# soon-yau/upgpt

Hardware: AMD Instinct MI355X
Metric: 256x256 images/sec, 50-step DDIM, bs=8/GPU; UNet MFMA util % (higher is better)
Workload: dtype f16; 1 GPU; BASELINE configs[1]: bs=8/GPU, 256x256 px (latent 4x32x32), 50-step DDIM eta=0, text-only cond [B,87,768], UNet(bbox.yaml) + VAE decode, EMA weights, no CFG; batch_per_gpu=8, ddim_steps=50, batches_in_flight_per_gpu=4, lane_hw_queues=measured, parallelism=replica-dp1, one all-gather of images per batch

## Files before the change

### upgpt_amd/csrc/attention.hip

```cpp
#include <stdlib.h>

#include "common.h"

namespace {

struct AttnArgs {
  const f16* q;
  const f16* k;
  const f16* vt;
  f16* o;
  int ldq, ldk, vt_ld, ldo;
  long qbs, kbs, obs;
  int heads, nq, nkv;
  float scale_log2;
  int causal;
};

__device__ __forceinline__ float raw_exp2(float x) { return __builtin_amdgcn_exp2f(x); }
__device__ __forceinline__ float max_over_key_groups(float x) {
  unsigned u = __float_as_uint(x);
  const auto a = __builtin_amdgcn_permlane32_swap(u, u, false, false);
  u = __float_as_uint(fmaxf(__uint_as_float(a[0]), __uint_as_float(a[1])));
  const auto b = __builtin_amdgcn_permlane16_swap(u, u, false, false);
  return fmaxf(__uint_as_float(b[0]), __uint_as_float(b[1]));
}
__device__ __forceinline__ float sum_over_key_groups(float x) {
  unsigned u = __float_as_uint(x);
  const auto a = __builtin_amdgcn_permlane32_swap(u, u, false, false);
  u = __float_as_uint(__uint_as_float(a[0]) + __uint_as_float(a[1]));
  const auto b = __builtin_amdgcn_permlane16_swap(u, u, false, false);
  return __uint_as_float(b[0]) + __uint_as_float(b[1]);
}
#define ATT_ONES ((f16x8){(f16)1.f, (f16)1.f, (f16)1.f, (f16)1.f, (f16)1.f, (f16)1.f, (f16)1.f, (f16)1.f})

template <int D, int QREG, int NS, int QT>
__device__ __forceinline__ void attn_tile(const AttnArgs& a, const f16* const* qrow, const bool* q_ok,
                                          const f16x8 (*qf)[QREG ? D / 32 : 1], const f16* kbase,
                                          const f16* vbase, int kb, int g, int c, f32x4 (*o)[D / 16], float* mrun,
                                          f32x4* lsum, int q0) {
  constexpr int KD = D / 32;
  constexpr int DT = D / 16;
  constexpr int NC = NS / 2;
  const f16x8 zero8 = {0, 0, 0, 0, 0, 0, 0, 0};
  f32x4 s[QT][NS];
  const f16* kp[NS];
#pragma unroll
  for (int t = 0; t < NS; ++t) {
    const int key = kb + 16 * t + c;
    kp[t] = kbase + (long)(key < a.nkv ? key : 0) * a.ldk;
#pragma unroll
    for (int u = 0; u < QT; ++u) s[u][t] = (f32x4){0.f, 0.f, 0.f, 0.f};
  }
#pragma unroll
  for (int kd = 0; kd < KD; ++kd) {
    f16x8 qv[QT];
#pragma unroll
    for (int u = 0; u < QT; ++u)
      qv[u] = QREG ? qf[u][kd] : (q_ok[u] ? *(const f16x8*)(qrow[u] + kd * 32) : zero8);
#pragma unroll
    for (int t = 0; t < NS; ++t) {
      const f16x8 kf = *(const f16x8*)(kp[t] + kd * 32);
#pragma unroll
      for (int u = 0; u < QT; ++u) s[u][t] = __builtin_amdgcn_mfma_f32_16x16x32_f16(kf, qv[u], s[u][t], 0, 0, 0);
    }
  }
  constexpr bool VPRE = (D <= 128);
  f16x4 vpre[VPRE ? DT * NC * 2 : 1];
  if (VPRE) {
#pragma unroll
    for (int i = 0; i < DT; ++i)
#pragma unroll
      for (int j = 0; j < NC; ++j) {
        const f16* vr = vbase + (long)i * 16 * a.vt_ld + kb + 32 * j;
        vpre[(i * NC + j) * 2] = *(const f16x4*)vr;
        vpre[(i * NC + j) * 2 + 1] = *(const f16x4*)(vr + 16);
      }
  }
  const float cs = a.scale_log2;
  f16x8 pf[QT][NC];
  const bool tail = kb + NS * 16 > a.nkv;
#pragma unroll
  for (int u = 0; u < QT; ++u) {
    if (tail || a.causal) {
      const int qlim = a.causal ? q0 + u * 16 + c : a.nkv;
#pragma unroll
      for (int t = 0; t < NS; ++t)
#pragma unroll
        for (int r = 0; r < 4; ++r) {
          const int key = kb + 16 * t + 4 * g + r;
          if (key >= a.nkv || key > qlim) s[u][t][r] = -INFINITY;
        }
    }
    float mx = -INFINITY;
#pragma unroll
    for (int t = 0; t < NS; ++t)
      mx = fmaxf(mx, fmaxf(fmaxf(s[u][t][0], s[u][t][1]), fmaxf(s[u][t][2], s[u][t][3])));
    mx = max_over_key_groups(mx);
    const float mnew = fmaxf(mrun[u], mx);
    if (__builtin_amdgcn_ballot_w64(mnew != mrun[u]) != 0) {
      const float alpha = raw_exp2((mrun[u] - mnew) * cs);
      lsum[u] *= alpha;
#pragma unroll
      for (int i = 0; i < DT; ++i) o[u][i] *= alpha;
    }
    mrun[u] = mnew;
    const float mc = -mnew * cs;
#pragma unroll
    for (int t = 0; t < NS; ++t)
#pragma unroll
      for (int r = 0; r < 4; ++r) pf[u][t >> 1][(t & 1) * 4 + r] = (f16)raw_exp2(fmaf(s[u][t][r], cs, mc));
  }
#pragma unroll
  for (int j = 0; j < NC; ++j)
#pragma unroll
    for (int u = 0; u < QT; ++u) lsum[u] = __builtin_amdgcn_mfma_f32_16x16x32_f16(ATT_ONES, pf[u][j], lsum[u], 0, 0, 0);
#pragma unroll
  for (int i = 0; i < DT; ++i)
#pragma unroll
    for (int j = 0; j < NC; ++j) {
      f16x4 va, vb;
      if (VPRE) {
        va = vpre[(i * NC + j) * 2];
        vb = vpre[(i * NC + j) * 2 + 1];
      } else {
        const f16* vr = vbase + (long)i * 16 * a.vt_ld + kb + 32 * j;
        va = *(const f16x4*)vr;
        vb = *(const f16x4*)(vr + 16);
      }
      const f16x8 vf = {va[0], va[1], va[2], va[3], vb[0], vb[1], vb[2], vb[3]};
#pragma unroll
      for (int u = 0; u < QT; ++u) o[u][i] = __builtin_amdgcn_mfma_f32_16x16x32_f16(vf, pf[u][j], o[u][i], 0, 0, 0);
    }
}

template <int D, int QREG, int QT>
__global__ __launch_bounds__(256) void attn_kernel(const AttnArgs a) {
  constexpr int KD = D / 32;
  constexpr int DT = D / 16;
  const int lane = threadIdx.x & 63;
  const int wave = threadIdx.x >> 6;
  const int g = lane >> 4, c = lane & 15;
  const int bh = blockIdx.x;
#ifndef UPK_NO_XCD_SAMPLE
  const int nb_ = gridDim.x / a.heads;
  const int b = bh % nb_;
  const int h = bh / nb_;
#else
  const int b = bh / a.heads;
  const int h = bh - b * a.heads;
#endif
  const int q0 = (blockIdx.y * (blockDim.x >> 6) + wave) * 16 * QT;
  if (q0 >= a.nq) return;
  const f16* kbase = a.k + b * a.kbs + h * D + g * 8;
  const f16* vbase = a.vt + ((long)(b * a.heads + h) * D + c) * a.vt_ld + g * 4;
  const f16x8 zero8 = {0, 0, 0, 0, 0, 0, 0, 0};

  const f16* qrow[QT];
  bool q_ok[QT];
  f16x8 qf[QT][QREG ? KD : 1];
  f32x4 o[QT][DT];
  float mrun[QT];
  f32x4 lsum[QT];
#pragma unroll
  for (int u = 0; u < QT; ++u) {
    const int qi = q0 + u * 16 + c;
    q_ok[u] = qi < a.nq;
    qrow[u] = a.q + b * a.qbs + (long)(q_ok[u] ? qi : 0) * a.ldq + h * D + g * 8;
    if (QREG) {
#pragma unroll
      for (int kd = 0; kd < KD; ++kd) qf[u][kd] = q_ok[u] ? *(const f16x8*)(qrow[u] + kd * 32) : zero8;
    }
#pragma unroll
    for (int i = 0; i < DT; ++i) o[u][i] = (f32x4){0.f, 0.f, 0.f, 0.f};
    mrun[u] = -INFINITY;
    lsum[u] = (f32x4){0.f, 0.f, 0.f, 0.f};
  }

  int kb = 0;
  if (D <= 128) {
    for (; kb + 64 <= (a.causal ? min(a.nkv, q0 + 16 * QT) : a.nkv); kb += 64)
      attn_tile<D, QREG, 4, QT>(a, qrow, q_ok, qf, kbase, vbase, kb, g, c, o, mrun, lsum, q0);
  }
  const int kend = a.causal ? min(a.nkv, q0 + 16 * QT) : a.nkv;
  for (; kb < kend; kb += 32) attn_tile<D, QREG, 2, QT>(a, qrow, q_ok, qf, kbase, vbase, kb, g, c, o, mrun, lsum, q0);

#pragma unroll
  for (int u = 0; u < QT; ++u) {
    const float inv = 1.0f / lsum[u][0];
    if (!q_ok[u]) continue;
    f16* orow = a.o + b * a.obs + (long)(q0 + u * 16 + c) * a.ldo + h * D + g * 4;
#pragma unroll
    for (int i = 0; i < DT; ++i) {
      f16x4 ov;
#pragma unroll
      for (int r = 0; r < 4; ++r) ov[r] = (f16)(o[u][i][r] * inv);
      *(f16x4*)(orow + i * 16) = ov;
    }
  }
}

struct QProj {
  const f16* x;
  const f16* w;
  const float* u;
  const float* bias;
  long xbs;
  int ldx, cq, ln_dim;
  float eps;
};

template <int D, int QT>
__global__ __launch_bounds__(256) void attn_qproj_kernel(const AttnArgs a, const QProj p) {
  constexpr int KD = D / 32;
  constexpr int DT = D / 16;
  constexpr int KC = 7;
  const int lane = threadIdx.x & 63;
  const int wave = threadIdx.x >> 6;
  const int g = lane >> 4, c = lane & 15;
  const int bh = blockIdx.y;
  const int b = bh / a.heads;
  const int h = bh - b * a.heads;
  const int q0 = (blockIdx.x * (blockDim.x >> 6) + wave) * 16 * QT;
  if (q0 >= a.nq) return;
  const f16* kbase = a.k + b * a.kbs + h * D + g * 8;
  const f16* vbase = a.vt + ((long)(b * a.heads + h) * D + c) * a.vt_ld + g * 4;

  const f16* qrow[QT];
  bool q_ok[QT];
  f16x8 qf[QT][KD];
  f32x4 o[QT][DT];
  float mrun[QT];
  f32x4 lsum[QT];
  {
    f32x4 qa[QT][DT];
    float s1[QT], s2[QT];
    const f16* xr[QT];
#pragma unroll
    for (int u = 0; u < QT; ++u) {
      const int qi = q0 + u * 16 + c;
      q_ok[u] = qi < a.nq;
      qrow[u] = nullptr;
      xr[u] = p.x + b * p.xbs + (long)(q_ok[u] ? qi : 0) * p.ldx + g * 8;
      s1[u] = s2[u] = 0.f;
#pragma unroll
      for (int i = 0; i < DT; ++i) qa[u][i] = (f32x4){0.f, 0.f, 0.f, 0.f};
    }
    const f16* wr = p.w + (long)(h * D + c) * p.cq + g * 8;
    const long wtile = (long)16 * p.cq;
    const f16x2 one2 = {(f16)1.f, (f16)1.f};
    for (int k0 = 0; k0 < p.cq; k0 += KC * 32) {
      f16x8 xv[QT][KC], wv[DT][KC];
#pragma unroll
      for (int kc = 0; kc < KC; ++kc) {
#pragma unroll
        for (int u = 0; u < QT; ++u) xv[u][kc] = *(const f16x8*)(xr[u] + k0 + kc * 32);
#pragma unroll
        for (int i = 0; i < DT; ++i) wv[i][kc] = *(const f16x8*)(wr + i * wtile + k0 + kc * 32);
      }
#pragma unroll
      for (int kc = 0; kc < KC; ++kc) {
#pragma unroll
        for (int u = 0; u < QT; ++u) {
#pragma unroll
          for (int hh = 0; hh < 4; ++hh) {
            const f16x2 xx = {xv[u][kc][2 * hh], xv[u][kc][2 * hh + 1]};
            s1[u] = __builtin_amdgcn_fdot2(xx, one2, s1[u], false);
            s2[u] = __builtin_amdgcn_fdot2(xx, xx, s2[u], false);
          }
#pragma unroll
          for (int i = 0; i < DT; ++i)
            qa[u][i] = __builtin_amdgcn_mfma_f32_16x16x32_f16(wv[i][kc], xv[u][kc], qa[u][i], 0, 0, 0);
        }
      }
    }
    const float inv_dim = 1.0f / (float)p.ln_dim;
    float mean[QT], rstd[QT];
#pragma unroll
    for (int u = 0; u < QT; ++u) {
      const float t1 = sum_over_key_groups(s1[u]), t2 = sum_over_key_groups(s2[u]);
      mean[u] = t1 * inv_dim;
      rstd[u] = rsqrtf(fmaxf(t2 * inv_dim - mean[u] * mean[u], 0.f) + p.eps);
    }
#pragma unroll
    for (int kd = 0; kd < KD; ++kd) {
      const int d0 = h * D + kd * 32 + g * 8;
      const f32x4 u0 = *(const f32x4*)(p.u + d0), u1 = *(const f32x4*)(p.u + d0 + 4);
      const f32x4 b0 = *(const f32x4*)(p.bias + d0), b1 = *(const f32x4*)(p.bias + d0 + 4);
#pragma unroll
      for (int u = 0; u < QT; ++u)
#pragma unroll
        for (int r = 0; r < 4; ++r) {
          qf[u][kd][r] = (f16)((qa[u][2 * kd][r] - mean[u] * u0[r]) * rstd[u] + b0[r]);
          qf[u][kd][4 + r] = (f16)((qa[u][2 * kd + 1][r] - mean[u] * u1[r]) * rstd[u] + b1[r]);
        }
    }
  }
#pragma unroll
  for (int u = 0; u < QT; ++u) {
#pragma unroll
    for (int i = 0; i < DT; ++i) o[u][i] = (f32x4){0.f, 0.f, 0.f, 0.f};
    mrun[u] = -INFINITY;
    lsum[u] = (f32x4){0.f, 0.f, 0.f, 0.f};
  }
  int kb = 0;
  for (; kb + 64 <= a.nkv; kb += 64) attn_tile<D, 1, 4, QT>(a, qrow, q_ok, qf, kbase, vbase, kb, g, c, o, mrun, lsum, q0);
  for (; kb < a.nkv; kb += 32) attn_tile<D, 1, 2, QT>(a, qrow, q_ok, qf, kbase, vbase, kb, g, c, o, mrun, lsum, q0);
#pragma unroll
  for (int u = 0; u < QT; ++u) {
    const float inv = 1.0f / lsum[u][0];
    if (!q_ok[u]) continue;
    f16* orow = a.o + b * a.obs + (long)(q0 + u * 16 + c) * a.ldo + h * D + g * 4;
#pragma unroll
    for (int i = 0; i < DT; ++i) {
      f16x4 ov;
#pragma unroll
      for (int r = 0; r < 4; ++r) ov[r] = (f16)(o[u][i][r] * inv);
      *(f16x4*)(orow + i * 16) = ov;
    }
  }
}

constexpr int ATT_VROW = 72;
__device__ __forceinline__ int att_swz(int row, int chunk) { return chunk ^ ((-(row >> 2)) & 3); }

template <int D, int QT>
__global__ __launch_bounds__(256) void attn_lds_kernel(const AttnArgs a) {
  constexpr int KD = D / 32;
  constexpr int DT = D / 16;
  __shared__ __attribute__((aligned(16))) f16 sk[2][KD * 64 * 32];
  __shared__ __attribute__((aligned(16))) f16 sv[2][D * ATT_VROW];
  const int tid = threadIdx.x;
  const int lane = tid & 63, wave = tid >> 6;
  const int g = lane >> 4, c = lane & 15;
  const int bh = blockIdx.x;
#ifndef UPK_NO_XCD_SAMPLE
  const int nb_ = gridDim.x / a.heads;
  const int b = bh % nb_;
  const int h = bh / nb_;
#else
  const int b = bh / a.heads;
  const int h = bh - b * a.heads;
#endif
  const int q0 = (blockIdx.y * 4 + wave) * 16 * QT;
  const f16x8 zero8 = {0, 0, 0, 0, 0, 0, 0, 0};

  bool q_ok[QT];
  f16x8 qf[QT][KD];
  f32x4 o[QT][DT];
  float mrun[QT];
  f32x4 lsum[QT];
#pragma unroll
  for (int u = 0; u < QT; ++u) {
    const int qi = q0 + u * 16 + c;
    q_ok[u] = qi < a.nq;
    const f16* qrow = a.q + b * a.qbs + (long)(q_ok[u] ? qi : 0) * a.ldq + h * D + g * 8;
#pragma unroll
    for (int kd = 0; kd < KD; ++kd) qf[u][kd] = q_ok[u] ? *(const f16x8*)(qrow + kd * 32) : zero8;
#pragma unroll
    for (int i = 0; i < DT; ++i) o[u][i] = (f32x4){0.f, 0.f, 0.f, 0.f};
    mrun[u] = -INFINITY;
    lsum[u] = (f32x4){0.f, 0.f, 0.f, 0.f};
  }
  const f16* ksrc = a.k + b * a.kbs + (long)(tid >> 2) * a.ldk + h * D + (tid & 3) * 8;
  const f16* vsrc = a.vt + ((long)(b * a.heads + h) * D + (tid >> 3)) * a.vt_ld + (tid & 7) * 8;
  const int kdst = (tid >> 2) * 32 + att_swz(tid >> 2, tid & 3) * 8;
  const int vdst = (tid >> 3) * ATT_VROW + (tid & 7) * 8;
  f16x8 kreg[KD], vreg[KD];
  auto fetch = [&](int kb) {
#pragma unroll
    for (int it = 0; it < KD; ++it) {
      kreg[it] = *(const f16x8*)(ksrc + (long)kb * a.ldk + it * 32);
      vreg[it] = *(const f16x8*)(vsrc + (long)it * 32 * a.vt_ld + kb);
    }
  };
  auto stash = [&](int buf) {
#pragma unroll
    for (int it = 0; it < KD; ++it) {
      *(f16x8*)(&sk[buf][it * 64 * 32 + kdst]) = kreg[it];
      *(f16x8*)(&sv[buf][it * 32 * ATT_VROW + vdst]) = vreg[it];
    }
  };
  const int ntiles = a.nkv >> 6;
  fetch(0);
  stash(0);
  __syncthreads();
  const float cs = a.scale_log2;
  const int kfrag = c * 32 + att_swz(c, g) * 8;
  for (int t = 0; t < ntiles; ++t) {
    const int buf = t & 1;
    if (t + 1 < ntiles) fetch((t + 1) << 6);
    f32x4 sc[QT][4];
#pragma unroll
    for (int tt = 0; tt < 4; ++tt)
#pragma unroll
      for (int u = 0; u < QT; ++u) sc[u][tt] = (f32x4){0.f, 0.f, 0.f, 0.f};
#pragma unroll
    for (int kd = 0; kd < KD; ++kd)
#pragma unroll
      for (int tt = 0; tt < 4; ++tt) {
        const f16x8 kf = *(const f16x8*)(&sk[buf][(kd * 64 + tt * 16) * 32 + kfrag]);
#pragma unroll
        for (int u = 0; u < QT; ++u) sc[u][tt] = __builtin_amdgcn_mfma_f32_16x16x32_f16(kf, qf[u][kd], sc[u][tt], 0, 0, 0);
      }
    f16x8 pf[QT][2];
#pragma unroll
    for (int u = 0; u < QT; ++u) {
      float mx = -INFINITY;
#pragma unroll
      for (int tt = 0; tt < 4; ++tt)
        mx = fmaxf(mx, fmaxf(fmaxf(sc[u][tt][0], sc[u][tt][1]), fmaxf(sc[u][tt][2], sc[u][tt][3])));
      mx = max_over_key_groups(mx);
      const float mnew = fmaxf(mrun[u], mx);
      if (__builtin_amdgcn_ballot_w64(mnew != mrun[u]) != 0) {
        const float alpha = raw_exp2((mrun[u] - mnew) * cs);
        lsum[u] *= alpha;
#pragma unroll
        for (int i = 0; i < DT; ++i) o[u][i] *= alpha;
      }
      mrun[u] = mnew;
      const float mc = -mnew * cs;
#pragma unroll
      for (int tt = 0; tt < 4; ++tt)
#pragma unroll
        for (int r = 0; r < 4; ++r) pf[u][tt >> 1][(tt & 1) * 4 + r] = (f16)raw_exp2(fmaf(sc[u][tt][r], cs, mc));
    }
#pragma unroll
    for (int j = 0; j < 2; ++j)
#pragma unroll
      for (int u = 0; u < QT; ++u) lsum[u] = __builtin_amdgcn_mfma_f32_16x16x32_f16(ATT_ONES, pf[u][j], lsum[u], 0, 0, 0);
#pragma unroll
    for (int i = 0; i < DT; ++i)
#pragma unroll
      for (int j = 0; j < 2; ++j) {
        const f16* vr = &sv[buf][(i * 16 + c) * ATT_VROW + 32 * j + 4 * g];
        const f16x4 va = *(const f16x4*)vr, vb = *(const f16x4*)(vr + 16);
        const f16x8 vf = {va[0], va[1], va[2], va[3], vb[0], vb[1], vb[2], vb[3]};
#pragma unroll
        for (int u = 0; u < QT; ++u) o[u][i] = __builtin_amdgcn_mfma_f32_16x16x32_f16(vf, pf[u][j], o[u][i], 0, 0, 0);
      }
    if (t + 1 < ntiles) stash(buf ^ 1);
    __syncthreads();
  }
#pragma unroll
  for (int u = 0; u < QT; ++u) {
    const float inv = 1.0f / lsum[u][0];
    if (!q_ok[u]) continue;
    f16* orow = a.o + b * a.obs + (long)(q0 + u * 16 + c) * a.ldo + h * D + g * 4;
#pragma unroll
    for (int i = 0; i < DT; ++i) {
      f16x4 ov;
#pragma unroll
      for (int r = 0; r < 4; ++r) ov[r] = (f16)(o[u][i][r] * inv);
      *(f16x4*)(orow + i * 16) = ov;
    }
  }
}

}

static int attn_waves_per_block(const upk_ctx* ctx, int bh, int n_q, int qt) {
  static const int wpb_env = getenv("UPK_ATTN_WPB") ? atoi(getenv("UPK_ATTN_WPB")) : 0;
  if (wpb_env == 1 || wpb_env == 2 || wpb_env == 4) return wpb_env;
  int wpb = 4;
  while (wpb > 1 && (long)bh * ((n_q + 16 * qt * wpb - 1) / (16 * qt * wpb)) < 2L * ctx->num_cus) wpb >>= 1;
  return wpb;
}

template <int D>
__global__ __launch_bounds__(256) void attn_wide_kernel(const AttnArgs a) {
  typedef __attribute__((address_space(3))) void* lds_ptr;
  typedef const __attribute__((address_space(1))) void* glb_ptr;
  constexpr int KD = D / 32, DT = D / 16;
  constexpr int KROW = D * 2 + 32;
  constexpr int KBYTES = 32 * KROW;
  constexpr int VBYTES = D * 64;
  constexpr int BUF = KBYTES + VBYTES;
  extern __shared__ __attribute__((aligned(16))) char smem[];
  const int lane = threadIdx.x & 63, wave = __builtin_amdgcn_readfirstlane(threadIdx.x >> 6);
  const int g = lane >> 4, c = lane & 15;
  const int b = blockIdx.x;
  const int q0 = (blockIdx.y * 4 + wave) * 16;
  const f16* kg = a.k + b * a.kbs;
  const f16* vg = a.vt + (long)b * D * a.vt_ld;
  auto issue = [&](int kb, int buf) {
    char* base = smem + buf * BUF;
#pragma unroll
    for (int i = 0; i < 8; ++i) {
      const int r = wave + 4 * i;
      const f16* src = kg + (long)(kb + r) * a.ldk + lane * 8;
      __builtin_amdgcn_global_load_lds((glb_ptr)src, (lds_ptr)(base + r * KROW), 16, 0, 0);
    }
#pragma unroll
    for (int i = 0; i < D / 64; ++i) {
      const int rb = (wave + 4 * i) * 16;
      const int row = rb + (lane >> 2), pc = (lane & 3) ^ ((row >> 2) & 3);
      const f16* src = vg + (long)row * a.vt_ld + kb + pc * 8;
      __builtin_amdgcn_global_load_lds((glb_ptr)src, (lds_ptr)(base + KBYTES + rb * 64), 16, 0, 0);
    }
  };
  issue(0, 0);
  const bool q_ok = q0 + c < a.nq;
  const f16* qrow = a.q + b * a.qbs + (long)(q_ok ? q0 + c : 0) * a.ldq + g * 8;
  f16x8 qf[KD];
#pragma unroll
  for (int kd = 0; kd < KD; ++kd) qf[kd] = q_ok ? *(const f16x8*)(qrow + kd * 32) : (f16x8){0, 0, 0, 0, 0, 0, 0, 0};
  f32x4 o[DT];
#pragma unroll
  for (int i = 0; i < DT; ++i) o[i] = (f32x4){0.f, 0.f, 0.f, 0.f};
  f32x4 lsum = {0.f, 0.f, 0.f, 0.f};
  float mrun = -INFINITY;
  const float cs = a.scale_log2;
  const int ntiles = a.nkv >> 5;
  const int vsw = (c >> 2) & 3;
  for (int t = 0; t < ntiles; ++t) {
    const int buf = t & 1;
    asm volatile("s_waitcnt vmcnt(0)" ::: "memory");
    __syncthreads();
    if (t + 1 < ntiles) issue((t + 1) << 5, buf ^ 1);
    const char* kt = smem + buf * BUF + c * KROW + g * 16;
    const char* vt = smem + buf * BUF + KBYTES + c * 64;
    f32x4 sc[2];
#pragma unroll
    for (int tt = 0; tt < 2; ++tt) {
      sc[tt] = (f32x4){0.f, 0.f, 0.f, 0.f};
#pragma unroll
      for (int kd = 0; kd < KD; ++kd) {
        const f16x8 kf = *(const f16x8*)(kt + tt * 16 * KROW + kd * 64);
        sc[tt] = __builtin_amdgcn_mfma_f32_16x16x32_f16(kf, qf[kd], sc[tt], 0, 0, 0);
      }
    }
    float mx = fmaxf(fmaxf(fmaxf(sc[0][0], sc[0][1]), fmaxf(sc[0][2], sc[0][3])),
                     fmaxf(fmaxf(sc[1][0], sc[1][1]), fmaxf(sc[1][2], sc[1][3])));
    mx = max_over_key_groups(mx);
    const float mnew = fmaxf(mrun, mx);
    if (__builtin_amdgcn_ballot_w64(mnew != mrun) != 0) {
      const float alpha = raw_exp2((mrun - mnew) * cs);
      lsum *= alpha;
#pragma unroll
      for (int i = 0; i < DT; ++i) o[i] *= alpha;
    }
    mrun = mnew;
    const float mc = -mnew * cs;
    f16x8 pf;
#pragma unroll
    for (int tt = 0; tt < 2; ++tt)
#pragma unroll
      for (int r = 0; r < 4; ++r) pf[tt * 4 + r] = (f16)raw_exp2(fmaf(sc[tt][r], cs, mc));
    lsum = __builtin_amdgcn_mfma_f32_16x16x32_f16(ATT_ONES, pf, lsum, 0, 0, 0);
#pragma unroll
    for (int i = 0; i < DT; ++i) {
      const char* vr = vt + i * 16 * 64 + (g & 1) * 8;
      const f16x4 va = *(const f16x4*)(vr + (((g >> 1) ^ vsw) << 4));
      const f16x4 vb = *(const f16x4*)(vr + (((2 + (g >> 1)) ^ vsw) << 4));
      const f16x8 vf = {va[0], va[1], va[2], va[3], vb[0], vb[1], vb[2], vb[3]};
      o[i] = __builtin_amdgcn_mfma_f32_16x16x32_f16(vf, pf, o[i], 0, 0, 0);
    }
  }
  if (!q_ok) return;
  const float inv = 1.0f / lsum[0];
  f16* orow = a.o + b * a.obs + (long)(q0 + c) * a.ldo + g * 4;
#pragma unroll
  for (int i = 0; i < DT; ++i) {
    f16x4 ov;
#pragma unroll
    for (int r = 0; r < 4; ++r) ov[r] = (f16)(o[i][r] * inv);
    *(f16x4*)(orow + i * 16) = ov;
  }
}

static int attention_impl(upk_ctx* ctx, const void* q, int ldq, long long qbs, const void* k, int ldk, long long kbs,
                          const void* vt, int vt_ld, void* out, int ldo, long long obs, int batch, int heads, int n_q,
                          int n_kv, int d, float scale, int causal, upk_stream stream_) {
  if (!ctx) return UPK_EINVAL;
  if (!q || !k || !vt || !out) return upk_fail(ctx, UPK_EINVAL, "attention: null pointer");
  if (batch <= 0 || heads <= 0 || n_q <= 0 || n_kv <= 0) return upk_fail(ctx, UPK_EINVAL, "attention: empty");
  if ((ldq & 7) || (ldk & 7) || (vt_ld & 3) || (ldo & 3) || vt_ld < ((n_kv + 31) & ~31))
    return upk_fail(ctx, UPK_EINVAL, "attention: ldq/ldk %% 8, vt_ld %% 4 and vt_ld >= round_up(n_kv,32) required");
  hipStream_t stream = (hipStream_t)stream_;
  AttnArgs a;
  a.q = (const f16*)q;
  a.k = (const f16*)k;
  a.vt = (const f16*)vt;
  a.o = (f16*)out;
  a.ldq = ldq;
  a.ldk = ldk;
  a.vt_ld = vt_ld;
  a.ldo = ldo;
  a.qbs = qbs;
  a.kbs = kbs;
  a.obs = obs;
  a.heads = heads;
  a.nq = n_q;
  a.nkv = n_kv;
  a.scale_log2 = scale * 1.4426950408889634f;
  a.causal = causal;
  if (causal && n_q != n_kv) return upk_fail(ctx, UPK_EINVAL, "attention: causal needs n_q == n_kv");
  static const int qt_env = getenv("UPK_ATTN_QT") ? atoi(getenv("UPK_ATTN_QT")) : 0;
  const int qt = qt_env ? qt_env : ((d <= 128 && (long)((n_q + 127) / 128) * batch * heads >= 4L * ctx->num_cus) ? 2 : 1);
  dim3 grid(batch * heads, (n_q + 64 * qt - 1) / (64 * qt)), block(256);
  upk_prof_scope prof(ctx, UPK_CLS_ATTN, stream);
  static const bool lds_off = getenv("UPK_ATTN_DIRECT") != nullptr;
  if (!lds_off && !causal && (d == 32 || d == 64) && n_kv >= 256 && (n_kv & 63) == 0 && (vt_ld & 7) == 0) {
    if (d == 32) {
      if (qt == 2) hipLaunchKernelGGL((attn_lds_kernel<32, 2>), grid, block, 0, stream, a);
      else hipLaunchKernelGGL((attn_lds_kernel<32, 1>), grid, block, 0, stream, a);
    } else {
      if (qt == 2) hipLaunchKernelGGL((attn_lds_kernel<64, 2>), grid, block, 0, stream, a);
      else hipLaunchKernelGGL((attn_lds_kernel<64, 1>), grid, block, 0, stream, a);
    }
    return upk_check_launch(ctx, "attention_lds");
  }
  {
    const int wpb = attn_waves_per_block(ctx, batch * heads, n_q, d <= 128 ? qt : 1);
    if (d <= 128) {
      grid = dim3(batch * heads, (n_q + 16 * qt * wpb - 1) / (16 * qt * wpb));
      block = dim3(64 * wpb);
    }
  }
#define UPK_ATTN(D_, QR_)                                                                         \
  if (qt == 2)                                                                                    \
    hipLaunchKernelGGL((attn_kernel<D_, QR_, (D_ <= 128 ? 2 : 1)>), grid, block, 0, stream, a);  \
  else                                                                                            \
    hipLaunchKernelGGL((attn_kernel<D_, QR_, 1>), grid, block, 0, stream, a);
  switch (d) {
    case 32: UPK_ATTN(32, 1) break;
    case 64: UPK_ATTN(64, 1) break;
    case 128: UPK_ATTN(128, 1) break;
    case 512:
      static const bool wide_off = getenv("UPK_ATTN_WIDE_OFF") != nullptr;
      if (heads == 1 && !causal && (n_kv & 31) == 0 && ldk >= 512 && !wide_off &&
          ((ldk | ldq | vt_ld) & 7) == 0 && ((kbs | qbs) & 7) == 0 &&
          (((uintptr_t)q | (uintptr_t)k | (uintptr_t)vt) & 15) == 0) {
        static unsigned long long wide_mask = 0;
        int rcw = upk_lds_attr_once(ctx, (const void*)attn_wide_kernel<512>, &wide_mask);
        if (rcw != UPK_OK) return rcw;
        const size_t lds = 2 * (32 * (512 * 2 + 32) + 512 * 64);
        hipLaunchKernelGGL((attn_wide_kernel<512>), dim3(batch, (n_q + 63) / 64), dim3(256), lds, stream, a);
        return upk_check_launch(ctx, "attention_wide");
      }
      [[fallthrough]];
    case 256: {
      const int wpb = attn_waves_per_block(ctx, batch * heads, n_q, 1);
      const dim3 g2(batch * heads, (n_q + 16 * wpb - 1) / (16 * wpb)), b2(64 * wpb);
      if (d == 256) hipLaunchKernelGGL((attn_kernel<256, 1, 1>), g2, b2, 0, stream, a);
      else hipLaunchKernelGGL((attn_kernel<512, 0, 1>), g2, b2, 0, stream, a);
      break;
    }
    default: return upk_fail(ctx, UPK_ESHAPE, "attention: head dim %d not in {32,64,128,256,512}", d);
  }
#undef UPK_ATTN
  return upk_check_launch(ctx, "attention");
}

extern "C" int upk_attention_f16(upk_ctx* ctx, const void* q, int ldq, long long qbs, const void* k, int ldk,
                                 long long kbs, const void* vt, int vt_ld, void* out, int ldo, long long obs,
                                 int batch, int heads, int n_q, int n_kv, int d, float scale, upk_stream stream) {
  return attention_impl(ctx, q, ldq, qbs, k, ldk, kbs, vt, vt_ld, out, ldo, obs, batch, heads, n_q, n_kv, d, scale, 0,
                        stream);
}

extern "C" int upk_attention_causal_f16(upk_ctx* ctx, const void* q, int ldq, long long qbs, const void* k, int ldk,
                                        long long kbs, const void* vt, int vt_ld, void* out, int ldo, long long obs,
                                        int batch, int heads, int n, int d, float scale, upk_stream stream) {
  return attention_impl(ctx, q, ldq, qbs, k, ldk, kbs, vt, vt_ld, out, ldo, obs, batch, heads, n, n, d, scale, 1, stream);
}

extern "C" int upk_attention_qproj_f16(upk_ctx* ctx, const void* x, int ldx, long long xbs, int cq, int ln_dim,
                                       float ln_eps, const void* wq, const float* wq_colsum, const float* wq_bias,
                                       const void* k, int ldk, long long kbs, const void* vt, int vt_ld, void* out,
                                       int ldo, long long obs, int batch, int heads, int n_q, int n_kv, int d,
                                       float scale, upk_stream stream_) {
  if (!ctx) return UPK_EINVAL;
  if (!x || !wq || !wq_colsum || !wq_bias || !k || !vt || !out) return upk_fail(ctx, UPK_EINVAL, "attention_qproj: null pointer");
  if (batch <= 0 || heads <= 0 || n_q <= 0 || n_kv <= 0) return upk_fail(ctx, UPK_EINVAL, "attention_qproj: empty");
  if ((ldx & 7) || (ldk & 7) || (vt_ld & 3) || (ldo & 3) || vt_ld < ((n_kv + 31) & ~31))
    return upk_fail(ctx, UPK_EINVAL, "attention_qproj: ldx/ldk %% 8, vt_ld %% 4 and vt_ld >= round_up(n_kv,32) required");
  if ((d != 32 && d != 64) || cq <= 0 || cq % 224 || ln_dim <= 0 || ln_dim > cq || ldx < cq)
    return upk_fail(ctx, UPK_ESHAPE, "attention_qproj: head dim %d / %d input channels outside {32,64} / 224*n", d, cq);
  hipStream_t stream = (hipStream_t)stream_;
  AttnArgs a;
  a.q = nullptr;
  a.k = (const f16*)k;
  a.vt = (const f16*)vt;
  a.o = (f16*)out;
  a.ldq = 0;
  a.ldk = ldk;
  a.vt_ld = vt_ld;
  a.ldo = ldo;
  a.qbs = 0;
  a.kbs = kbs;
  a.obs = obs;
  a.heads = heads;
  a.nq = n_q;
  a.nkv = n_kv;
  a.scale_log2 = scale * 1.4426950408889634f;
  a.causal = 0;
  QProj p;
  p.x = (const f16*)x;
  p.w = (const f16*)wq;
  p.u = wq_colsum;
  p.bias = wq_bias;
  p.xbs = xbs;
  p.ldx = ldx;
  p.cq = cq;
  p.ln_dim = ln_dim;
  p.eps = ln_eps;
  upk_prof_scope prof(ctx, UPK_CLS_ATTN, stream);
  const int qt = d == 32 ? 2 : 1;
  const int wpb = attn_waves_per_block(ctx, batch * heads, n_q, qt);
  const dim3 grid((n_q + 16 * qt * wpb - 1) / (16 * qt * wpb), batch * heads), block(64 * wpb);
  if (d == 32) hipLaunchKernelGGL((attn_qproj_kernel<32, 2>), grid, block, 0, stream, a, p);
  else hipLaunchKernelGGL((attn_qproj_kernel<64, 1>), grid, block, 0, stream, a, p);
  return upk_check_launch(ctx, "attention_qproj");
}
```

Before: 98.94 images/s.

## Software-pipeline LDS attention kernel with swizzled V layout and multi-tile stages

Restructures the LDS flash-attention kernel so the next tile's QK scores and V fragments are loaded while the current tile's PV accumulation runs, using ping-pong register sets. For D=32 it stages two 64-key tiles per barrier (four LDS slots) to halve synchronisation. V in LDS now uses an XOR-swizzled 64-wide row instead of padded 72-wide rows, so each V fragment is a single 16-byte read. It also lowers the threshold for picking QT=2 on the LDS path. Costs are higher register pressure and more LDS for D=32, which may reduce occupancy.

Result: no change. 98.76 images/s (median of 2 runs) (-0.2%).

```diff
diff --git a/upgpt_amd/csrc/attention.hip b/upgpt_amd/csrc/attention.hip
--- a/upgpt_amd/csrc/attention.hip
+++ b/upgpt_amd/csrc/attention.hip
@@ -320,15 +320,17 @@
   }
 }
 
-constexpr int ATT_VROW = 72;
+constexpr int ATT_VROW = 64;
 __device__ __forceinline__ int att_swz(int row, int chunk) { return chunk ^ ((-(row >> 2)) & 3); }
 
 template <int D, int QT>
 __global__ __launch_bounds__(256) void attn_lds_kernel(const AttnArgs a) {
   constexpr int KD = D / 32;
   constexpr int DT = D / 16;
-  __shared__ __attribute__((aligned(16))) f16 sk[2][KD * 64 * 32];
-  __shared__ __attribute__((aligned(16))) f16 sv[2][D * ATT_VROW];
+  constexpr int TPS = D == 32 ? 2 : 1;
+  constexpr int NSLOT = 2 * TPS;
+  __shared__ __attribute__((aligned(16))) f16 sk[NSLOT][KD * 64 * 32];
+  __shared__ __attribute__((aligned(16))) f16 sv[NSLOT][D * ATT_VROW];
   const int tid = threadIdx.x;
   const int lane = tid & 63, wave = tid >> 6;
   const int g = lane >> 4, c = lane & 15;
@@ -364,32 +366,46 @@
   const f16* ksrc = a.k + b * a.kbs + (long)(tid >> 2) * a.ldk + h * D + (tid & 3) * 8;
   const f16* vsrc = a.vt + ((long)(b * a.heads + h) * D + (tid >> 3)) * a.vt_ld + (tid & 7) * 8;
   const int kdst = (tid >> 2) * 32 + att_swz(tid >> 2, tid & 3) * 8;
-  const int vdst = (tid >> 3) * ATT_VROW + (tid & 7) * 8;
-  f16x8 kreg[KD], vreg[KD];
-  auto fetch = [&](int kb) {
-#pragma unroll
-    for (int it = 0; it < KD; ++it) {
-      kreg[it] = *(const f16x8*)(ksrc + (long)kb * a.ldk + it * 32);
-      vreg[it] = *(const f16x8*)(vsrc + (long)it * 32 * a.vt_ld + kb);
+  const int vrow = tid >> 3, vj = (tid & 7) >> 2, vw = (tid & 3) * 8;
+  const int vq = 4 * vj + (vw & 15) / 4, vh = vw >> 4;
+  const int vdst0 = vrow * ATT_VROW + ((vq ^ (vrow & 7)) << 3) + 4 * vh;
+  const int vdst1 = vrow * ATT_VROW + (((vq + 1) ^ (vrow & 7)) << 3) + 4 * vh;
+  const int ntiles = a.nkv >> 6;
+  const int nstages = (ntiles + TPS - 1) / TPS;
+  f16x8 kreg[TPS][KD], vreg[TPS][KD];
+  auto fetch = [&](int st) {
+#pragma unroll
+    for (int j = 0; j < TPS; ++j) {
+      const int kb = (st * TPS + j) << 6;
+      if (TPS == 1 || kb < a.nkv) {
+#pragma unroll
+        for (int it = 0; it < KD; ++it) {
+          kreg[j][it] = *(const f16x8*)(ksrc + (long)kb * a.ldk + it * 32);
+          vreg[j][it] = *(const f16x8*)(vsrc + (long)it * 32 * a.vt_ld + kb);
+        }
+      }
     }
   };
-  auto stash = [&](int buf) {
-#pragma unroll
-    for (int it = 0; it < KD; ++it) {
-      *(f16x8*)(&sk[buf][it * 64 * 32 + kdst]) = kreg[it];
-      *(f16x8*)(&sv[buf][it * 32 * ATT_VROW + vdst]) = vreg[it];
+  auto stash = [&](int st) {
+#pragma unroll
+    for (int j = 0; j < TPS; ++j) {
+      const int tl = st * TPS + j;
+      if (TPS == 1 || tl < ntiles) {
+        const int slot = tl % NSLOT;
+#pragma unroll
+        for (int it = 0; it < KD; ++it) {
+          *(f16x8*)(&sk[slot][it * 64 * 32 + kdst]) = kreg[j][it];
+          const f16x8 vv = vreg[j][it];
+          *(f16x4*)(&sv[slot][it * 32 * ATT_VROW + vdst0]) = (f16x4){vv[0], vv[1], vv[2], vv[3]};
+          *(f16x4*)(&sv[slot][it * 32 * ATT_VROW + vdst1]) = (f16x4){vv[4], vv[5], vv[6], vv[7]};
+        }
+      }
     }
   };
-  const int ntiles = a.nkv >> 6;
-  fetch(0);
-  stash(0);
-  __syncthreads();
   const float cs = a.scale_log2;
   const int kfrag = c * 32 + att_swz(c, g) * 8;
-  for (int t = 0; t < ntiles; ++t) {
-    const int buf = t & 1;
-    if (t + 1 < ntiles) fetch((t + 1) << 6);
-    f32x4 sc[QT][4];
+  auto load_tile = [&](int tl, f32x4 (&sc)[QT][4], f16x8 (&vf)[DT][2]) {
+    const int slot = tl % NSLOT;
 #pragma unroll
     for (int tt = 0; tt < 4; ++tt)
 #pragma unroll
@@ -398,11 +414,19 @@
     for (int kd = 0; kd < KD; ++kd)
 #pragma unroll
       for (int tt = 0; tt < 4; ++tt) {
-        const f16x8 kf = *(const f16x8*)(&sk[buf][(kd * 64 + tt * 16) * 32 + kfrag]);
+        const f16x8 kf = *(const f16x8*)(&sk[slot][(kd * 64 + tt * 16) * 32 + kfrag]);
 #pragma unroll
         for (int u = 0; u < QT; ++u) sc[u][tt] = __builtin_amdgcn_mfma_f32_16x16x32_f16(kf, qf[u][kd], sc[u][tt], 0, 0, 0);
       }
-    f16x8 pf[QT][2];
+#pragma unroll
+    for (int i = 0; i < DT; ++i)
+#pragma unroll
+      for (int j = 0; j < 2; ++j) {
+        const int row = i * 16 + c;
+        vf[i][j] = *(const f16x8*)(&sv[slot][row * ATT_VROW + (((4 * j + g) ^ (c & 7)) << 3)]);
+      }
+  };
+  auto update_max = [&](const f32x4 (&sc)[QT][4]) {
 #pragma unroll
     for (int u = 0; u < QT; ++u) {
       float mx = -INFINITY;
@@ -418,7 +442,13 @@
         for (int i = 0; i < DT; ++i) o[u][i] *= alpha;
       }
       mrun[u] = mnew;
-      const float mc = -mnew * cs;
+    }
+  };
+  auto accumulate = [&](const f32x4 (&sc)[QT][4], const f16x8 (&vf)[DT][2]) {
+    f16x8 pf[QT][2];
+#pragma unroll
+    for (int u = 0; u < QT; ++u) {
+      const float mc = -mrun[u] * cs;
 #pragma unroll
       for (int tt = 0; tt < 4; ++tt)
 #pragma unroll
@@ -431,15 +461,40 @@
 #pragma unroll
     for (int i = 0; i < DT; ++i)
 #pragma unroll
-      for (int j = 0; j < 2; ++j) {
-        const f16* vr = &sv[buf][(i * 16 + c) * ATT_VROW + 32 * j + 4 * g];
-        const f16x4 va = *(const f16x4*)vr, vb = *(const f16x4*)(vr + 16);
-        const f16x8 vf = {va[0], va[1], va[2], va[3], vb[0], vb[1], vb[2], vb[3]};
-#pragma unroll
-        for (int u = 0; u < QT; ++u) o[u][i] = __builtin_amdgcn_mfma_f32_16x16x32_f16(vf, pf[u][j], o[u][i], 0, 0, 0);
-      }
-    if (t + 1 < ntiles) stash(buf ^ 1);
-    __syncthreads();
+      for (int j = 0; j < 2; ++j)
+#pragma unroll
+        for (int u = 0; u < QT; ++u) o[u][i] = __builtin_amdgcn_mfma_f32_16x16x32_f16(vf[i][j], pf[u][j], o[u][i], 0, 0, 0);
+  };
+  auto step = [&](int t, const f32x4 (&sc)[QT][4], const f16x8 (&vf)[DT][2], f32x4 (&sn)[QT][4], f16x8 (&vn)[DT][2]) {
+    if ((t + 1) % TPS == 0) {
+      const int st = (t + 1) / TPS;
+      stash(st);
+      __syncthreads();
+      if (st + 1 < nstages) fetch(st + 1);
+    }
+    load_tile(t + 1, sn, vn);
+    accumulate(sc, vf);
+    update_max(sn);
+  };
+
+  f32x4 sa[QT][4], sb[QT][4];
+  f16x8 va[DT][2], vb[DT][2];
+  fetch(0);
+  stash(0);
+  __syncthreads();
+  if (nstages > 1) fetch(1);
+  load_tile(0, sa, va);
+  update_max(sa);
+  int t = 0;
+  for (; t + 2 < ntiles; t += 2) {
+    step(t, sa, va, sb, vb);
+    step(t + 1, sb, vb, sa, va);
+  }
+  if (t + 1 < ntiles) {
+    step(t, sa, va, sb, vb);
+    accumulate(sb, vb);
+  } else {
+    accumulate(sa, va);
   }
 #pragma unroll
   for (int u = 0; u < QT; ++u) {
@@ -596,11 +651,13 @@
   a.causal = causal;
   if (causal && n_q != n_kv) return upk_fail(ctx, UPK_EINVAL, "attention: causal needs n_q == n_kv");
   static const int qt_env = getenv("UPK_ATTN_QT") ? atoi(getenv("UPK_ATTN_QT")) : 0;
-  const int qt = qt_env ? qt_env : ((d <= 128 && (long)((n_q + 127) / 128) * batch * heads >= 4L * ctx->num_cus) ? 2 : 1);
+  int qt = qt_env ? qt_env : ((d <= 128 && (long)((n_q + 127) / 128) * batch * heads >= 4L * ctx->num_cus) ? 2 : 1);
   dim3 grid(batch * heads, (n_q + 64 * qt - 1) / (64 * qt)), block(256);
   upk_prof_scope prof(ctx, UPK_CLS_ATTN, stream);
   static const bool lds_off = getenv("UPK_ATTN_DIRECT") != nullptr;
   if (!lds_off && !causal && (d == 32 || d == 64) && n_kv >= 256 && (n_kv & 63) == 0 && (vt_ld & 7) == 0) {
+    if (!qt_env) qt = (long)((n_q + 127) / 128) * batch * heads >= 2L * ctx->num_cus ? 2 : 1;
+    grid.y = (n_q + 64 * qt - 1) / (64 * qt);
     if (d == 32) {
       if (qt == 2) hipLaunchKernelGGL((attn_lds_kernel<32, 2>), grid, block, 0, stream, a);
       else hipLaunchKernelGGL((attn_lds_kernel<32, 1>), grid, block, 0, stream, a);
```
